# mbhall88/drprg

Measured on AMD Instinct MI355X. Metric: reads/sec (+ achieved HBM GB/s) predicting on mtb index, 1/2/4/8 GPUs, higher is better.
Workload: dtype u32

## Files before the change

### drprg_amd/_lib.py

```python
import ctypes as C
import os

_HERE = os.path.dirname(os.path.abspath(__file__))
LIB_PATH = os.environ.get("DRPRG_HIP_LIB") or os.path.join(_HERE, "lib", "libdrprg_hip.so")
PANDORA_EXE = os.path.join(_HERE, "bin", "pandora")


class MapOpts(C.Structure):
    _fields_ = [
        ("max_diff", C.c_int32),
        ("error_rate", C.c_double),
        ("min_cluster_size", C.c_uint32),
        ("illumina", C.c_int32),
        ("genome_size", C.c_uint64),
        ("genotyping_error_rate", C.c_double),
        ("kernel", C.c_int32),
        ("binomial", C.c_int32),
    ]


class AnnotateOpts(C.Structure):
    _fields_ = [
        ("min_covg", C.c_int32), ("max_covg", C.c_int32),
        ("min_strand_bias", C.c_float), ("min_gt_conf", C.c_float), ("min_frs", C.c_float),
# ... 70 lines not shown
    "drprg_hip_genotype": (C.c_int, [C.c_void_p, C.c_char_p, C.c_char_p, C.c_char_p]),
    "drprg_hip_genotype_info": (C.c_int, [C.c_void_p, C.POINTER(C.c_uint32)]),
    "drprg_hip_discover": (C.c_int, [C.c_void_p, C.c_char_p, C.c_char_p, C.c_char_p, C.POINTER(C.c_uint32)]),
    "drprg_hip_discover_reads": (C.c_int, [C.c_void_p, C.c_char_p, C.c_char_p, C.c_char_p, C.c_char_p, C.c_int, C.POINTER(C.c_uint32)]),
    "drprg_hip_update_prg": (C.c_int, [C.c_void_p, C.c_char_p, C.POINTER(C.c_uint32)]),
    "drprg_hip_update_prg_from_paths": (C.c_int, [C.c_void_p, C.c_char_p, C.c_char_p, C.POINTER(C.c_uint32)]),
    "drprg_hip_save_coverage": (C.c_int, [C.c_void_p, C.c_char_p, C.c_char_p]),
    "drprg_hip_load_coverage": (C.c_int, [C.c_void_p, C.c_char_p, C.c_char_p, C.POINTER(C.c_uint64)]),
    "drprg_hip_allele_stats": (C.c_int, [C.c_void_p, C.c_void_p, C.c_uint32, C.c_uint32, C.c_void_p, C.POINTER(C.c_double)]),
    "drprg_hip_genotype_site": (C.c_int, [C.c_void_p, C.c_void_p, C.c_void_p, C.c_uint32, C.c_double, C.c_double, C.c_void_p,
                                          C.POINTER(C.c_int32), C.POINTER(C.c_double)]),
    "drprg_hip_genotype_alleles": (C.c_int, [C.c_void_p, C.c_char_p]),
    "drprg_hip_estimate_parameters": (C.c_int, [C.c_void_p, C.c_uint64, C.c_uint64, C.c_uint64, C.c_uint32, C.c_int, C.c_double, C.c_int,
                                               C.POINTER(C.c_double)]),
    "drprg_hip_kmer_log_prob": (C.c_int, [C.c_int, C.c_double, C.c_double, C.c_double, C.c_uint32, C.c_uint32, C.c_uint32, C.POINTER(C.c_float)]),
    "drprg_hip_prob_threshold": (C.c_int, [C.c_void_p, C.c_uint64, C.POINTER(C.c_int)]),
    "drprg_hip_max_path": (C.c_int, [C.c_void_p, C.c_uint32, C.c_void_p, C.c_int, C.c_uint32, C.c_void_p, C.c_uint64, C.POINTER(C.c_uint64)]),
    "drprg_hip_path_base_coverage": (C.c_int, [C.c_void_p, C.c_uint32, C.c_void_p, C.c_uint64, C.c_void_p, C.c_void_p, C.c_uint64,
                                              C.POINTER(C.c_uint64)]),
    "drprg_hip_path_coverage_too_low": (C.c_int, [C.c_void_p, C.c_uint64, C.c_uint32]),
    "drprg_hip_coverage_model": (C.c_int, [C.c_void_p, C.POINTER(C.c_double)]),
    "drprg_hip_index_sizes": (C.c_int, [C.c_void_p, C.POINTER(C.c_uint64)]),
    "drprg_hip_filter_selfcheck": (C.c_int, [C.c_void_p, C.POINTER(C.c_uint64)]),
    "drprg_hip_device_tables": (C.c_int, [C.c_void_p, C.POINTER(C.c_uint64)]),
    "drprg_hip_index_export": (C.c_int, [C.c_void_p] + [C.c_void_p] * 7),
    "drprg_hip_prg_nodes": (C.c_int, [C.c_void_p, C.c_uint32, C.c_void_p, C.c_void_p, C.c_uint32, C.POINTER(C.c_uint32),
                                      C.POINTER(C.c_uint32)]),
    "drprg_hip_annotate": (C.c_int, [C.c_char_p, C.c_char_p, C.c_char_p, C.POINTER(AnnotateOpts), C.c_char_p, C.c_size_t]),
    "drprg_hip_vcf_to_bcf": (C.c_int, [C.c_char_p, C.c_char_p, C.c_char_p, C.c_size_t]),
    "drprg_hip_report_json": (C.c_int, [C.c_char_p, C.c_char_p, C.c_char_p, C.c_char_p, C.c_int, C.c_char_p, C.c_char_p,
                                        C.c_size_t]),
    "drprg_hip_kernel_timing": (C.c_int, [C.c_void_p, C.c_int, C.c_int, C.POINTER(C.c_double), C.POINTER(C.c_uint64)]),
    "drprg_hip_filter_schedule": (C.c_int, [C.c_void_p, C.POINTER(C.c_uint64)]),
    "drprg_hip_buffer_info": (C.c_int, [C.c_void_p, C.POINTER(C.c_uint64)]),
}


def load():
    if not os.path.exists(LIB_PATH):
        raise ImportError(
            f"{LIB_PATH} is missing: build the HIP extension first (`make` at the repo root or "
            "`python -c 'import __graft_entry__ as g; g.build()'`). There is no CPU fallback.")
    try:
        import torch
    except Exception:
        pass
# ... 10 lines not shown
```

### drprg_amd/csrc/capi.cpp

```cpp
#include <set>
#include <atomic>
#include <mutex>
#include <thread>
#include <fstream>
#include <cstdio>
#include "../../include/drprg_hip.h"
#include "fastx.h"
#include "genotype.h"
#include "bam.h"
#include "ingest.h"
#include "pgunzip.h"
#include "denovo.h"
#include "mapper.h"
#include "rccl_dyn.h"
#include "pack.h"
#include "read_qual_piece.h"
#include <algorithm>
#include <cstdlib>
#include <cstring>
#include <fcntl.h>
#include <functional>
#include <sys/mman.h>
#include <sys/stat.h>
#include <unistd.h>
// ... 1378 lines not shown
        al[a].gaps = gaps[a];
    }
    int g = 0;
    genotype_site(al, e, eps, g, *gt_conf);
    *gt = g;
    for (uint32_t a = 0; a < n_alleles; ++a) likelihood[a] = al[a].likelihood;
    return DRPRG_OK;
}

int drprg_hip_genotype_info(const drprg_hip_ctx* ctx, uint32_t out[4])
{
    if (!ctx || !out) return DRPRG_EINVAL;
    std::memcpy(out, ctx->ginfo, sizeof ctx->ginfo);
    return DRPRG_OK;
}

int drprg_hip_filter_selfcheck(const drprg_hip_ctx* ctx, uint64_t out[8])
{
    if (!ctx || !out) return DRPRG_EINVAL;
    ctx->index.filter_selfcheck(out);
    return DRPRG_OK;
}

int drprg_hip_index_sizes(const drprg_hip_ctx* ctx, uint64_t sizes[5])
{
    if (!ctx || !sizes) return DRPRG_EINVAL;
    const FlatIndex& f = ctx->index.flat;
    sizes[0] = f.keys.size();
    sizes[1] = f.rec_prg.size();
    sizes[2] = ctx->index.prgs.size();
    sizes[3] = f.total_knodes();
    sizes[4] = f.slot_key.size();
    return DRPRG_OK;
}

int drprg_hip_index_export(const drprg_hip_ctx* ctx, uint64_t* keys, uint32_t* rec_off, uint32_t* rec_prg, uint32_t* rec_knode,
    uint8_t* rec_strand, uint32_t* prg_min_path_len, uint32_t* prg_knode_base)
{
    if (!ctx) return DRPRG_EINVAL;
    const FlatIndex& f = ctx->index.flat;
    if (keys) std::memcpy(keys, f.keys.data(), f.keys.size() * sizeof(uint64_t));
    if (rec_off) std::memcpy(rec_off, f.rec_off.data(), f.rec_off.size() * sizeof(uint32_t));
    if (rec_prg) std::memcpy(rec_prg, f.rec_prg.data(), f.rec_prg.size() * sizeof(uint32_t));
    if (rec_knode) std::memcpy(rec_knode, f.rec_knode_global.data(), f.rec_knode_global.size() * sizeof(uint32_t));
    if (rec_strand) std::memcpy(rec_strand, f.rec_strand.data(), f.rec_strand.size());
    if (prg_min_path_len) std::memcpy(prg_min_path_len, f.min_path_len.data(), f.min_path_len.size() * sizeof(uint32_t));
// ... 246 lines not shown
```

### drprg_amd/csrc/common.h

```cpp
#pragma once
#include <cstdlib>
#include <cstdint>
#include <cstdio>
#include <stdexcept>
#include <string>
#include <vector>

namespace drprg {

struct Error : std::runtime_error {
    int code;
    Error(int c, const std::string& m) : std::runtime_error(m), code(c) {}
};

enum : int {
    DRPRG_OK = 0,
    DRPRG_EINVAL = -22,
    DRPRG_ENOENT = -2,
    DRPRG_EIO = -5,
    DRPRG_ENOMEM = -12,
    DRPRG_ENODEV = -19,
    DRPRG_EOVERFLOW = -75,
    DRPRG_EFORMAT = -84,
    DRPRG_ENODATA = -61,
// ... 10 lines not shown
    key = key ^ key >> 14;
    key = ((key + (key << 2)) + (key << 4)) & mask;
    key = key ^ key >> 28;
    key = (key + (key << 31)) & mask;
    return key;
}

inline int nt4(unsigned char c)
{
    switch (c) {
    case 'A': case 'a': return 0;
    case 'C': case 'c': return 1;
    case 'G': case 'g': return 2;
    case 'T': case 't': return 3;
    default: return 4;
    }
}

constexpr uint32_t BLOOM_C0 = 0xC2B2AFu;
constexpr uint32_t BLOOM_C1 = 0x9E3779u;
constexpr uint32_t BLOOM_C2 = 0x85EBCA6Bu;
constexpr uint32_t BLOOM_CR = 0xC2B2AE35u;
constexpr uint32_t BLOOMR_WBITS = 14;
constexpr uint32_t MID_BITMAP_WORDS = 1u << 19;
constexpr uint32_t MID_C_MAX_WBITS = 17;
inline uint32_t rc12_code(uint32_t x)
{
    uint32_t r = 0;
    for (int i = 0; i < 12; ++i) r |= (((x >> (2 * i)) & 3u) ^ 2u) << (2 * (11 - i));
    return r;
}
inline uint32_t canon12_code(uint32_t x)
{
    x &= 0xFFFFFFu;
    const uint32_t r = rc12_code(x);
    return x < r ? x : r;
}

inline bool canonical_kmer_hash(const char* s, int k, uint64_t& h, bool& strand)
{
    const uint64_t mask = kmer_mask(k);
    uint64_t f = 0, r = 0;
    for (int i = 0; i < k; ++i) {
        int c = nt4((unsigned char)s[i]);
        if (c > 3) return false;
        f = (f << 2) | (uint64_t)c;
// ... 24 lines not shown
```

### drprg_amd/csrc/index.cpp

```cpp
#include "index.h"
#include <algorithm>
#include <atomic>
#include <cerrno>
#include <cmath>
#include <cstdlib>
#include <fstream>
#include <sstream>
#include <sys/stat.h>
#include <thread>

namespace drprg {

static std::string dir_of(const std::string& p)
{
    size_t s = p.find_last_of('/');
    return s == std::string::npos ? std::string(".") : p.substr(0, s);
}

std::string PrgIndex::idx_path(const std::string& prg_file, int w, int k)
{
    return prg_file + ".k" + std::to_string(k) + ".w" + std::to_string(w) + ".idx";
}

std::string PrgIndex::gfa_path(const std::string& prg_file, const std::string& name, int w, int k)
// ... 13 lines not shown
    w = w_;
    k = k_;
    prgs = load_prg_file(prg_file);
    kgs.assign(prgs.size(), KmerGraph());
    std::atomic<size_t> next { 0 };
    std::string err;
    std::atomic<bool> failed { false };
    auto work = [&]() {
        for (size_t i; (i = next.fetch_add(1)) < prgs.size();) {
            try {
                kgs[i].build(prgs[i], w, k);
            } catch (const std::exception& e) {
                if (!failed.exchange(true)) err = e.what();
            }
        }
    };
    int nt = std::max(1, std::min<int>(threads, (int)prgs.size()));
    std::vector<std::thread> pool;
    for (int t = 1; t < nt; ++t) pool.emplace_back(work);
    work();
    for (auto& t : pool) t.join();
    if (failed) throw Error(DRPRG_EFORMAT, err);
    flatten(sw);
}

void PrgIndex::flatten(const Switches& sw)
{
    FlatIndex& f = flat;
    f = FlatIndex();
    f.knode_base.assign(prgs.size() + 1, 0);
    f.min_path_len.assign(prgs.size(), 0);
    struct Rec {
        uint64_t key;
        uint32_t prg, knode;
        uint8_t strand;
    };
    std::vector<Rec> recs;
    for (size_t p = 0; p < prgs.size(); ++p) {
        f.knode_base[p + 1] = f.knode_base[p] + (uint32_t)kgs[p].nodes.size();
        f.min_path_len[p] = kgs[p].shortest_path_length;
        const auto& nodes = kgs[p].nodes;
        for (size_t i = 1; i + 1 < nodes.size(); ++i)
            recs.push_back(Rec { nodes[i].hash, (uint32_t)p, nodes[i].id, (uint8_t)(nodes[i].strand ? 1 : 0) });
    }
    std::sort(recs.begin(), recs.end(), [](const Rec& a, const Rec& b) {
        if (a.key != b.key) return a.key < b.key;
// ... 50 lines not shown
        const uint32_t max_wbits = level0 ? MAX_WBITS - 1 : MAX_WBITS;
        uint32_t wbits = 8;
        while (wbits < max_wbits && (size_t(1) << wbits) * 5 < entries * 4) ++wbits;
        f.bloom_wbits = wbits;
        f.bloom.assign(size_t(1) << wbits, 0);
        const uint32_t wmask = (1u << wbits) - 1;
        const uint32_t kmask = (1u << (2 * k)) - 1;
        if (level0) {
            f.bloom0_wbits = L0_WBITS;
            f.bloom0.assign(size_t(1) << L0_WBITS, 0);
            f.bloom0f.assign(size_t(1) << L0_WBITS, 0);
            f.bloomr.assign(size_t(1) << BLOOMR_WBITS, 0);
        }
        const uint32_t wmask0 = (1u << L0_WBITS) - 1;
        for_each_code([&](uint32_t code) {
            const uint32_t x = code & kmask & 0xFFFFFFu;
            const uint32_t h = (uint32_t)((uint64_t)x * BLOOM_C1);
            f.bloom[(h >> 18) & wmask] |= (1u << (31 - (h & 31))) | (1u << (31 - ((h >> 8) & 31))) | (1u << (31 - ((x >> 16) & 31)));
            const uint32_t h2 = code * BLOOM_C2;
            f.bloom[h2 >> (32 - wbits)] |= (1u << (h2 & 31)) | (1u << ((h2 >> 5) & 31)) | (1u << ((h2 >> 10) & 31));
            if (level0) {
                const uint32_t hr = code * BLOOM_CR;
                f.bloomr[hr >> (32 - BLOOMR_WBITS)] |= (1u << (hr & 31)) | (1u << ((hr >> 5) & 31)) | (1u << ((hr >> 10) & 31)) | (1u << ((hr >> 15) & 31));
                const uint32_t hs = code * BLOOM_C2;
                f.bloom0f[hr >> (32 - L0_WBITS)] |= (1u << (hr & 31)) | (1u << ((hr >> 5) & 31)) | (1u << ((hr >> 10) & 31)) | (1u << (hs >> 27))
                    | (1u << ((hs >> 22) & 31)) | (1u << ((hs >> 17) & 31));
            }
            if (level0)
                for (int o = 0; o < 4; ++o) {
                    const uint32_t y = (code >> (2 * o)) & 0xFFFFFFu;
                    const uint32_t g = (uint32_t)((uint64_t)y * BLOOM_C0);
                    const uint32_t bits0 = (1u << (31 - (g & 31))) | (1u << (31 - ((g >> 8) & 31))) | (1u << (31 - ((y >> 16) & 31)));
                    f.bloom0[(g >> 17) & wmask0] |= bits0;
                    f.bloom0f[(g >> 17) & wmask0] |= bits0;
                }
        });
        if (level0) {
            uint32_t cw = 10;
            while (cw < MID_C_MAX_WBITS && (size_t(4) << cw) < 4 * entries) ++cw;
            f.blkc_wbits = cw;
            f.blkc.assign(size_t(4) << cw, 0);
            for_each_code([&](uint32_t code) {
                const uint32_t h = code * BLOOM_CR;
                for (int o = 0; o < 4; ++o) {
                    const uint32_t key = (code >> (2 * o)) & 0xFFFFFFu;
                    const uint32_t blk = (uint32_t)((uint64_t)key * BLOOM_C0) >> (32 - cw);
                    uint32_t* b = &f.blkc[(size_t)blk * 4];
                    b[0] |= 1u << (h >> 27);
                    b[1] |= 1u << ((h >> 22) & 31);
                    b[2] |= 1u << ((h >> 17) & 31);
                    b[3] |= 1u << ((h >> 12) & 31);
                }
            });
        }
    } else if (k == 15 && entries > 0 && recs.size() <= sw.mid_max_records) {
        f.mid_bitmap.assign(MID_BITMAP_WORDS, 0);
        for_each_code([&](uint32_t code) {
// ... 82 lines not shown
        out[4] = fill(f.mid0);
        out[5] = fill(f.mid_bitmap);
        out[6] = fill(f.midc);
        return;
    }
    if (!f.bloom_wbits) return;
    const uint32_t wmask = (1u << f.bloom_wbits) - 1, kmask = (1u << (2 * k)) - 1, wmask0 = f.bloom0_wbits ? (1u << f.bloom0_wbits) - 1 : 0;
    auto three = [](uint32_t word, uint32_t h, uint32_t x) {
        return ((word << (h & 31)) & (word << ((h >> 8) & 31)) & (word << ((x >> 16) & 31))) >> 31;
    };
    auto check = [&](uint32_t code) {
        ++out[0];
        if (f.bloom0_wbits) {
            bool any_miss = false;
            for (int o = 0; o < 4; ++o) {
                const uint32_t y = (code >> (2 * o)) & 0xFFFFFFu;
                const uint32_t g = (uint32_t)((uint64_t)y * BLOOM_C0);
                any_miss |= !three(f.bloom0[(g >> 17) & wmask0], g, y);
            }
            out[1] += any_miss;
            const uint32_t hr = code * BLOOM_CR, word = f.bloomr[hr >> (32 - BLOOMR_WBITS)];
            out[3] += !((word >> (hr & 31)) & (word >> ((hr >> 5) & 31)) & (word >> ((hr >> 10) & 31)) & (word >> ((hr >> 15) & 31)) & 1u);
            bool miss_f = false;
            for (int o = 0; o < 4; ++o) {
                const uint32_t y = (code >> (2 * o)) & 0xFFFFFFu;
                const uint32_t g = (uint32_t)((uint64_t)y * BLOOM_C0);
                miss_f |= !three(f.bloom0f[(g >> 17) & wmask0], g, y);
            }
            const uint32_t wf = f.bloom0f[hr >> (32 - f.bloom0_wbits)];
            const uint32_t hs = code * BLOOM_C2;
            miss_f |= !((wf >> (hr & 31)) & (wf >> ((hr >> 5) & 31)) & (wf >> ((hr >> 10) & 31)) & (wf >> (hs >> 27)) & (wf >> ((hs >> 22) & 31))
                & (wf >> ((hs >> 17) & 31)) & 1u);
            bool miss_blk = false;
            if (f.blkc_wbits)
                for (int o = 0; o < 4; ++o) {
                    const uint32_t key = (code >> (2 * o)) & 0xFFFFFFu;
                    const uint32_t* b = &f.blkc[(size_t)((uint32_t)((uint64_t)key * BLOOM_C0) >> (32 - f.blkc_wbits)) * 4];
                    miss_blk |= !((b[0] >> (hr >> 27)) & (b[1] >> ((hr >> 22) & 31)) & (b[2] >> ((hr >> 17) & 31)) & (b[3] >> ((hr >> 12) & 31)) & 1u);
                }
            out[7] += miss_f || miss_blk;
        }
        const uint32_t x = code & kmask & 0xFFFFFFu;
        const uint32_t h = (uint32_t)((uint64_t)x * BLOOM_C1);
        const uint32_t h2 = code * BLOOM_C2, w2 = f.bloom[h2 >> (32 - f.bloom_wbits)];
        const bool l1 = three(f.bloom[(h >> 18) & wmask], h, x);
        const bool l2 = (w2 >> (h2 & 31)) & (w2 >> ((h2 >> 5) & 31)) & (w2 >> ((h2 >> 10) & 31)) & 1u;
        out[2] += !(l1 && l2);
    };
    for (size_t p = 0; p < prgs.size(); ++p) {
        const auto& nodes = kgs[p].nodes;
        for (size_t i = 1; i + 1 < nodes.size(); ++i) {
            const std::string s = kpath_sequence(prgs[p], nodes[i].path);
            uint32_t fw = 0, rc = 0;
            for (int j = 0; j < k; ++j) {
                const uint32_t c = ((uint32_t)(unsigned char)s[(size_t)j] >> 1) & 3u;
                fw |= c << (2 * j);
                rc |= (c ^ 2u) << (2 * (k - 1 - j));
            }
            check(fw);
            check(rc);
        }
    }
    auto fill = [](const std::vector<uint32_t>& v) -> uint64_t {
        uint64_t bits = 0;
        for (uint32_t w : v) bits += (uint64_t)__builtin_popcount(w);
        return v.empty() ? 0 : bits * 1000 / (32 * (uint64_t)v.size());
    };
    out[4] = fill(f.bloom0);
    out[5] = fill(f.bloom);
    out[6] = fill(f.bloomr);
}

void PrgIndex::save(const std::string& prg_file) const
{
    std::string kdir = dir_of(prg_file) + "/kmer_prgs";
    if (mkdir(kdir.c_str(), 0777) != 0 && errno != EEXIST) throw Error(DRPRG_EIO, "cannot create " + kdir);
    for (size_t p = 0; p < prgs.size(); ++p) kgs[p].save_gfa(gfa_path(prg_file, prgs[p].name, w, k), prgs[p]);
    std::ofstream out(idx_path(prg_file, w, k));
    if (!out) throw Error(DRPRG_EIO, "cannot write " + idx_path(prg_file, w, k));
    const FlatIndex& f = flat;
    auto path_string = [&](uint32_t prg, uint32_t node) {
        std::ostringstream os;
        const KPath& kp = kgs[prg].nodes[node].path;
        os << kp.size() << "{";
        for (const PathPiece& pp : kp) {
            const uint32_t base = prgs[prg].nodes[pp.node].start;
            os << "[" << base + pp.off_start << ", " << base + pp.off_end << ")";
        }
        os << "}";
        return os.str();
    };
    out << f.keys.size() << "\n";
    for (size_t i = 0; i < f.keys.size(); ++i) {
// ... 66 lines not shown
```

### drprg_amd/csrc/index.h

```cpp
#pragma once
#include "kmergraph.h"
#include "switches.h"

namespace drprg {

struct MiniRecord {
    uint32_t prg;
    uint32_t knode;
    uint8_t strand;
};

struct FlatIndex {
    std::vector<uint64_t> keys;
    std::vector<uint32_t> rec_off;
    std::vector<uint32_t> rec_prg, rec_knode_global;
    std::vector<uint8_t> rec_strand;
    std::vector<uint32_t> knode_base;
    std::vector<uint32_t> min_path_len;
    uint32_t table_bits = 0;
    std::vector<uint64_t> slot_key;
    std::vector<uint32_t> slot_off, slot_cnt;
    uint32_t bloom_wbits = 0;
    std::vector<uint32_t> bloom;
    uint32_t bloom0_wbits = 0;
    std::vector<uint32_t> bloom0;
    std::vector<uint32_t> bloom0f;
    std::vector<uint32_t> bloomr;
    uint32_t midc_wbits = 0, mid0_bits = 0;
    std::vector<uint32_t> mid0, mid_bitmap, midc;
    uint32_t blkc_wbits = 0;
    std::vector<uint32_t> blkc;
    uint32_t total_knodes() const { return knode_base.empty() ? 0 : knode_base.back(); }
};

struct PrgIndex {
    int w = 0, k = 0;
    std::vector<LocalGraph> prgs;
    std::vector<KmerGraph> kgs;
    FlatIndex flat;
    void filter_selfcheck(uint64_t out[8]) const;

    static void check_wk(int w, int k);
    static void build_and_save(const std::string& prg_file, int w, int k, int threads, const Switches& sw);
    void build(const std::string& prg_file, int w, int k, int threads, const Switches& sw);
    void load(const std::string& prg_file, int w, int k, const Switches& sw);
    void save(const std::string& prg_file) const;

    static std::string idx_path(const std::string& prg_file, int w, int k);
    static std::string gfa_path(const std::string& prg_file, const std::string& name, int w, int k);

private:
    void flatten(const Switches& sw);
};

inline uint32_t table_slot(uint64_t key, uint32_t bits, bool narrow)
{
    if (narrow) return ((uint32_t)key * 0x9E3779B1u) >> (32 - bits);
    return (uint32_t)((key * 0x9E3779B97F4A7C15ULL) >> (64 - bits));
}

}
```

### drprg_amd/csrc/sketch_filter.hip

```cpp
#include "filter_common.h"
#include <algorithm>
#include <cstdint>
#include <type_traits>

namespace drprg {
namespace dev {

__device__ inline uint32_t pack16le(const uint4& in)
{
    constexpr uint32_t W = 0x40100401u;
    const uint32_t p0 = __builtin_amdgcn_udot4(in.x & 0x06060606u, W, 0u, false), p1 = __builtin_amdgcn_udot4(in.y & 0x06060606u, W, 0u, false);
    const uint32_t p2 = __builtin_amdgcn_udot4(in.z & 0x06060606u, W, 0u, false), p3 = __builtin_amdgcn_udot4(in.w & 0x06060606u, W, 0u, false);
    return ((p0 | (p1 << 8) | (p2 << 16)) >> 1) | (p3 << 23);
}


typedef __attribute__((address_space(3))) const uint32_t lds_cu32;
__device__ __forceinline__ uint32_t lds_at(uint32_t byte_addr) { return *(lds_cu32*)(uintptr_t)byte_addr; }
__device__ __forceinline__ uint32_t bloom_test(uint32_t word, uint32_t h, uint32_t x)
{
    uint32_t t2;
    asm("v_lshlrev_b32_sdwa %0, %1, %2 dst_sel:DWORD dst_unused:UNUSED_PAD src0_sel:BYTE_1 src1_sel:DWORD" : "=v"(t2) : "v"(h), "v"(word));
    return (word << (h & 31)) & t2 & (word << ((x >> 16) & 0xFF));
}

__device__ __forceinline__ uint32_t canon12_dev(uint32_t x)
{
    const uint32_t m = x & 0xFFFFFFu;
    const uint32_t r = __builtin_bitreverse32(x);
    const uint32_t rc = ((r >> 9) & 0x555555u) | (~(r >> 7) & 0xAAAAAAu);
    return m < rc ? m : rc;
}

template <bool SHORT_K, bool LEVEL0, bool FUSED = false, int MID = 0, bool PACKED = false>
__global__ __launch_bounds__(FT_THREADS) void sketch_filter_kernel(SketchArgs a, FilterWork fw)
{
    static_assert(FUSED == LEVEL0, "the level-0 form runs its second stage in this kernel");
    static_assert(MID == 0 || (LEVEL0 && FUSED), "the middle tier is a variant of the level-0 form with the second stage inside");
    extern __shared__ uint32_t s_dyn[];
    constexpr int G = filter_positions_per_lane(LEVEL0, PACKED), WPOS = 63 * G, NW = G / 16, NG = G / 4;
    constexpr uint32_t L12_BASE = LEVEL0 ? FT_L0_WORDS * 4u : 0u;
    constexpr bool CANON = MID == 1 || MID == 3;
    auto group_key = [](uint32_t x) -> uint32_t {
        if constexpr (CANON) return canon12_dev(x);
        else return x;
    };
    (void)group_key;
    constexpr uint32_t STAGE_RECORDS = 128, STAGE_CAP = STAGE_RECORDS - 1, STAGE_BASE_WORDS = FT_L0_WORDS;

    const int tid = threadIdx.x, lane = tid & 63;
    const int k = a.k;
    const int64_t n_bases = (int64_t)a.n_bases;
    const uint32_t n_words = 1u << fw.bloom_wbits;
    const uint32_t amask = (n_words - 1) << 2;
    const uint32_t amask0 = ((1u << fw.bloom0_wbits) - 1) << 2;
    const uint32_t kmask = (k < 16) ? ((1u << (2 * k)) - 1) : 0xFFFFFFFFu;
    const uint32_t kmask24 = kmask & 0xFFFFFFu;
    const int sh_w = 32 - (int)fw.bloom_wbits;
    const uint32_t sh_c = 32u - fw.midc_wbits;
    (void)sh_c;

    auto fill = [&](uint32_t lds_word0, const uint32_t* __restrict__ from, uint32_t n) {
        const uint4* __restrict__ src = reinterpret_cast<const uint4*>(from);
        uint4* dst = reinterpret_cast<uint4*>(s_dyn + lds_word0);
        for (uint32_t i = tid; i < n / 4; i += FT_THREADS) dst[i] = src[i];
    };
    if constexpr (LEVEL0) {
        constexpr int ROUNDS = FT_L0_WORDS / 4 / FT_THREADS;
        const uint4* __restrict__ src = reinterpret_cast<const uint4*>(fw.bloom0);
        uint4* dst = reinterpret_cast<uint4*>(s_dyn);
        uint4 v[ROUNDS];
#pragma unroll
        for (int r = 0; r < ROUNDS; ++r) v[r] = src[tid + r * FT_THREADS];
#pragma unroll
        for (int r = 0; r < ROUNDS; ++r) dst[tid + r * FT_THREADS] = v[r];
    }
    if (!LEVEL0) fill(L12_BASE / 4, fw.bloom, n_words);
    if (tid == 0 && (uint32_t)(uintptr_t)(__attribute__((address_space(3))) uint32_t*)s_dyn != 0u) atomicOr(a.overflow, 8u);
// ... 131 lines not shown
                        ra = stage[ia];                                                                                               \
                        ba = reinterpret_cast<const uint4*>(fw.midc)[(uint32_t)__umul24(group_key(__funnelshift_r(ra.z, ra.w, 6)), BLOOM_C0) >> sh_c];  \
                    }                                                                                                                 \
                    if (ib < lcnt) {                                                                                                  \
                        rb = stage[ib];                                                                                               \
                        bb = reinterpret_cast<const uint4*>(fw.midc)[(uint32_t)__umul24(group_key(__funnelshift_r(rb.z, rb.w, 6)), BLOOM_C0) >> sh_c]; \
                    }                                                                                                                 \
                    uint32_t ca = 0, cb = 0;                                                                                          \
                    DRPRG_BLOCK_TEST(ra, ba, ca);                            \
                    DRPRG_STAGE2_APPEND(ra, ca);                                                                                      \
                    if (c0 + 64 < lcnt) {                                                                           \
                        DRPRG_BLOCK_TEST(rb, bb, cb);                                                                                 \
                        DRPRG_STAGE2_APPEND(rb, cb);                                                                                  \
                    }                                                                                                                 \
                }                                                                                                                     \
            } else {                                                                                                                  \
                for (uint32_t c0 = 0; c0 < lcnt; c0 += 64) {                                                                          \
                    const uint32_t ri = c0 + (uint32_t)lane;                                                                          \
                    uint32_t cs = 0;                                                                                                  \
                    uint4 r = make_uint4(0, 0, 0, 0);                                                                                 \
                    if (ri < lcnt) {                                                                                                  \
                        r = stage[ri];                                                                                                \
                                                                     \
                        uint32_t hq[4], h2q[4], wq[4];                                                                                \
                        _Pragma("unroll") for (int q = 0; q < 4; ++q) {                                                               \
                            const uint32_t f = (q ? __funnelshift_r(r.z, r.w, 2 * q) : r.z) & kmask;                                  \
                            hq[q] = f * BLOOM_CR;                                                                                     \
                            h2q[q] = f * BLOOM_C2;                                                                                    \
                            wq[q] = lds_at((hq[q] >> 17) << 2);                                                                       \
                        }                                                                                                             \
                        __builtin_amdgcn_sched_barrier(0);      \
                        _Pragma("unroll") for (int q = 0; q < 4; ++q)                                                                 \
                            cs |= ((wq[q] >> (hq[q] & 31)) & (wq[q] >> ((hq[q] >> 5) & 31)) & (wq[q] >> ((hq[q] >> 10) & 31)) & (wq[q] >> (h2q[q] >> 27)) \
                                      & (wq[q] >> ((h2q[q] >> 22) & 31)) & (wq[q] >> ((h2q[q] >> 17) & 31)) & 1u) << q;               \
                    }                                                                                                                 \
                    DRPRG_STAGE2_APPEND(r, cs);                                                                                       \
                }                                                                                                                     \
            }                                                                                                                         \
            __builtin_amdgcn_wave_barrier();                                                                                          \
            lcnt = 0;                                                                                                                 \
        }                                                                                                                             \
    } while (0)
    auto close_slice = [&]() {
        if constexpr (FUSED) DRPRG_SECOND_STAGE();
        if (lane == 0) {
            const uint32_t kept = wcur < cap_cur ? wcur : cap_cur;
            fw.slice_count[slice] = kept;
            fw.slice_base[slice] = base_cur;
            fw.slice_cap[slice] = cap_cur;
            if (wcur > cap_cur) atomicOr(a.overflow, 4u);
            if (kept) atomicAdd(&fw.super_count[slice / FT_SUPER], kept);
        }
    };

    auto process = [&](uint32_t t, const Pair& p) {
        uint32_t wv[NW + 1];
        if constexpr (PACKED) {
            wv[0] = p.x;
            wv[1] = p.y;
            if constexpr (NW == 4) {
                wv[2] = p.z;
                wv[3] = p.w;
            }
        } else {
            wv[0] = pack16le(p.a);
            wv[1] = pack16le(p.b);
        }
        wv[NW] = __builtin_amdgcn_update_dpp(0u, wv[0], 0x130 , 0xF, 0xF, true);
        const uint32_t wa = wv[0], wb = wv[1], wc = wv[2];
        (void)wa; (void)wb; (void)wc;
        if constexpr (LEVEL0) {
            uint32_t grp = 0, xs[NG], hs[NG], ws[NG];
#pragma unroll
            for (int g = 0; g < NG; ++g) {
                const int j = 4 * g + 3;
                const uint32_t lo = wv[j >> 4], hi = wv[(j >> 4) + 1];
                xs[g] = __builtin_amdgcn_alignbit(hi, lo, 2 * (j & 15));
                if constexpr (CANON) xs[g] = canon12_dev(xs[g]);
                hs[g] = __umul24(xs[g], BLOOM_C0);
                ws[g] = lds_at((hs[g] >> 15) & amask0);
            }
#pragma unroll
            for (int g = NG - 1; g >= 0; --g)
                grp = __builtin_amdgcn_alignbit(grp, MID == 1 ? ws[g] << (hs[g] & 31) : bloom_test(ws[g], hs[g], xs[g]), 31);
            grp &= lane_keep;
            if constexpr (CANON) {
                uint32_t bw[NG];
#pragma unroll
                for (int g = 0; g < NG; ++g) {
                    bw[g] = 0;
                    if (grp & (1u << g)) bw[g] = fw.mid_bitmap[xs[g] >> 5];
                }
                uint32_t keep = 0;
#pragma unroll
                for (int g = 0; g < NG; ++g) keep |= ((bw[g] >> (xs[g] & 31)) & 1u) << g;
                grp &= keep;
            }
            const uint32_t cnt = (uint32_t)__popc(grp);
            const uint64_t b0 = __ballot(cnt & 1u), b1 = __ballot(cnt & 2u), b2 = __ballot(cnt & 4u), b3 = __ballot(cnt & 8u);
            const uint64_t b4 = NG > 8 ? __ballot(cnt & 16u) : 0ull;
            if (b0 | b1 | b2 | b3 | b4) {
                auto below = [&](uint64_t m) { return __builtin_amdgcn_mbcnt_hi((uint32_t)(m >> 32), __builtin_amdgcn_mbcnt_lo((uint32_t)m, 0u)); };
                auto lanes_below = [&]() { return below(b0) + 2u * below(b1) + 4u * below(b2) + 8u * below(b3) + (NG > 8 ? 16u * below(b4) : 0u); };
                const uint32_t total = (uint32_t)(__popcll(b0) + 2 * __popcll(b1) + 4 * __popcll(b2) + 8 * __popcll(b3) + (NG > 8 ? 16 * __popcll(b4) : 0));
                const uint64_t base = (uint64_t)t * WPOS + (uint64_t)lane * G;
                auto record = [&](int g) {
                    const int q = g >> 2;
// ... 355 lines not shown
```

### drprg_amd/pandora.py

```python
import ctypes as C
import os
import re

import numpy as np

from ._lib import MapOpts, lib

MTB_GENOME_SIZE = 4411532


class DependencyError(RuntimeError):

    def __init__(self, kind, message, code=0):
        super().__init__(f"{kind}: {message}")
        self.kind = kind
        self.code = code


def _check(rc, ctx=None):
    if rc != 0:
        msg = lib.drprg_hip_last_error(ctx)
        raise DependencyError("ProcessError", (msg or b"").decode() or f"error {rc}", code=-rc)


# ... 246 lines not shown
    def load_coverage(self, path, tag):
        rc = lib.drprg_hip_load_coverage(self._h, os.fsencode(path), tag.encode(), None)
        if rc == -2:
            return False
        _check(rc, self._h)
        return True

    def genotype_alleles(self, out_tsv):
        _check(lib.drprg_hip_genotype_alleles(self._h, os.fsencode(out_tsv)), self._h)
        out = {}
        for line in open(out_tsv):
            if line.startswith("#"):
                continue
            chrom, pos, a, n, nodes = line.rstrip("\n").split("\t")
            out[(chrom, int(pos), int(a))] = np.array([int(x) for x in nodes.split(",") if x], dtype=np.int64)
        return out

    def filter_selfcheck(self):
        out = (C.c_uint64 * 8)()
        _check(lib.drprg_hip_filter_selfcheck(self._h, out), self._h)
        names = ("codes", "level0_false_negatives", "level12_false_negatives", "stage2_false_negatives", "level0_fill_permille",
                 "level12_fill_permille", "stage2_fill_permille", "shared_array_false_negatives")
        return dict(zip(names, (int(x) for x in out)))

    def table_tier(self):
        out = (C.c_uint64 * 6)()
        _check(lib.drprg_hip_device_tables(self._h, out), self._h)
        return dict(pbloom_words=int(out[0]), table_bytes=int(out[1]), lds_filter_bytes=int(out[2]), kernel=int(out[3]),
                    l2_filter_bytes=int(out[4]), sketch_form=int(out[5]))

    def export_index(self):
        keys = np.zeros(self.n_keys, dtype=np.uint64)
        rec_off = np.zeros(self.n_keys + 1, dtype=np.uint32)
        rec_prg = np.zeros(self.n_records, dtype=np.uint32)
        rec_knode = np.zeros(self.n_records, dtype=np.uint32)
        rec_strand = np.zeros(self.n_records, dtype=np.uint8)
        min_path_len = np.zeros(self.n_prgs, dtype=np.uint32)
        knode_base = np.zeros(self.n_prgs + 1, dtype=np.uint32)
        _check(lib.drprg_hip_index_export(self._h, _ptr(keys), _ptr(rec_off), _ptr(rec_prg), _ptr(rec_knode), _ptr(rec_strand),
                                          _ptr(min_path_len), _ptr(knode_base)), self._h)
        return dict(keys=keys, rec_off=rec_off, rec_prg=rec_prg, rec_knode=rec_knode, rec_strand=rec_strand,
                    min_path_len=min_path_len, knode_base=knode_base)

    def prg_nodes(self, prg):
        n, ns = C.c_uint32(), C.c_uint32()
        _check(lib.drprg_hip_prg_nodes(self._h, prg, None, None, 0, C.byref(n), C.byref(ns)), self._h)
# ... 174 lines not shown
```

### include/drprg_hip.h

```cpp
#ifndef DRPRG_HIP_H
#define DRPRG_HIP_H

#include <stddef.h>
#include <stdint.h>

#ifdef __cplusplus
extern "C" {
#endif

typedef struct drprg_hip_ctx drprg_hip_ctx;

#define DRPRG_HIP_MAP_OPTS_SIZE 48
typedef struct drprg_hip_map_opts {
    int32_t max_diff;
    double error_rate;
    uint32_t min_cluster_size;
    int32_t illumina;
    uint64_t genome_size;
    double genotyping_error_rate;
    int32_t kernel;
    int32_t binomial;
} drprg_hip_map_opts;

int drprg_hip_index(const char* prg_file, int w, int k, int threads);
// ... 67 lines not shown
int drprg_hip_resident_info(drprg_hip_ctx* ctx, uint64_t out[4]);
int drprg_hip_subsample(drprg_hip_ctx* ctx, uint64_t target_bases, uint64_t seed, uint64_t out[4]);
int drprg_hip_set_ordered_ingest(drprg_hip_ctx* ctx, int on);
int drprg_hip_subsample_flags(drprg_hip_ctx* ctx, uint8_t* flags, uint64_t n);
int drprg_hip_set_read_filter(drprg_hip_ctx* ctx, uint64_t min_len, uint64_t max_len, uint32_t min_qual_milli);
int drprg_hip_read_filter_info(drprg_hip_ctx* ctx, uint64_t out[8]);
int drprg_hip_read_filter_device(drprg_hip_ctx* ctx, const void* d_qual, uint32_t qual_bias, const void* d_offsets, uint64_t n_reads, uint64_t n_bases,
    void* d_sums, void* d_flags, uint64_t out[4], void* hip_stream);
int drprg_hip_select_reads(drprg_hip_ctx* ctx, const uint64_t* anchors, uint64_t n_anchors, uint32_t A, uint64_t window_bytes, uint8_t* bases,
    uint64_t bases_cap, uint64_t* offsets, uint64_t* ids, uint64_t reads_cap, uint64_t out[2]);

int drprg_hip_update_prg(drprg_hip_ctx* ctx, const char* out_prg, uint32_t* n_applied);
int drprg_hip_update_prg_from_paths(drprg_hip_ctx* ctx, const char* denovo_paths, const char* out_prg, uint32_t* n_applied);

int drprg_hip_save_coverage(drprg_hip_ctx* ctx, const char* path, const char* tag);
int drprg_hip_load_coverage(drprg_hip_ctx* ctx, const char* path, const char* tag, uint64_t counters[8]);

int drprg_hip_allele_stats(const uint32_t* fwd, const uint32_t* rev, uint32_t n, uint32_t min_kmer_covg, uint32_t out[6], double* gaps);
int drprg_hip_genotype_site(const uint32_t* mean_fwd, const uint32_t* mean_rev, const double* gaps, uint32_t n_alleles, double e,
    double eps, double* likelihood, int32_t* gt, double* gt_conf);
int drprg_hip_genotype_alleles(drprg_hip_ctx* ctx, const char* out_tsv);

int drprg_hip_filter_selfcheck(const drprg_hip_ctx* ctx, uint64_t out[8]);
int drprg_hip_estimate_parameters(const uint32_t* kmer_covg, uint64_t n, uint64_t clusters, uint64_t loci, uint32_t global_covg, int k,
    double e_rate, int bin, double out[10]);
int drprg_hip_kmer_log_prob(int use_bin, double nb_p, double nb_r, double bin_p, uint32_t fwd, uint32_t rev, uint32_t locus_reads, float* out);
int drprg_hip_prob_threshold(const float* logp, uint64_t n, int* out);
int drprg_hip_max_path(const drprg_hip_ctx* ctx, uint32_t prg, const float* logp, int thresh, uint32_t max_kmers_to_average, uint32_t* path,
    uint64_t cap, uint64_t* n_path);
int drprg_hip_path_base_coverage(const drprg_hip_ctx* ctx, uint32_t prg, const uint32_t* path, uint64_t n_path, const uint32_t* covg2,
    uint32_t* out, uint64_t cap, uint64_t* n_out);
int drprg_hip_path_coverage_too_low(const uint32_t* base_covg, uint64_t n, uint32_t global_covg);
int drprg_hip_coverage_model(const drprg_hip_ctx* ctx, double out[12]);

int drprg_hip_index_sizes(const drprg_hip_ctx* ctx, uint64_t sizes[5]);
int drprg_hip_index_export(const drprg_hip_ctx* ctx, uint64_t* keys, uint32_t* rec_off, uint32_t* rec_prg,
    uint32_t* rec_knode, uint8_t* rec_strand, uint32_t* prg_min_path_len, uint32_t* prg_knode_base);

int drprg_hip_device_tables(drprg_hip_ctx* ctx, uint64_t out[6]);

int drprg_hip_prg_nodes(const drprg_hip_ctx* ctx, uint32_t prg, uint32_t* starts, uint32_t* ends, uint32_t cap,
    uint32_t* n_nodes, uint32_t* n_sites);

typedef struct drprg_hip_annotate_opts {
    int32_t min_covg, max_covg;
    float min_strand_bias, min_gt_conf, min_frs;
// ... 23 lines not shown
```

Baseline: 21.69 billion.

## Widen shared level-0/stage-2 bloom array to 64-bit blocks

```diff
diff --git a/drprg_amd/_lib.py b/drprg_amd/_lib.py
--- a/drprg_amd/_lib.py
+++ b/drprg_amd/_lib.py
@@ -116,6 +116,8 @@
     "drprg_hip_coverage_model": (C.c_int, [C.c_void_p, C.POINTER(C.c_double)]),
     "drprg_hip_index_sizes": (C.c_int, [C.c_void_p, C.POINTER(C.c_uint64)]),
     "drprg_hip_filter_selfcheck": (C.c_int, [C.c_void_p, C.POINTER(C.c_uint64)]),
+    "drprg_hip_filter_sample": (C.c_int, [C.c_void_p, C.c_uint64, C.c_uint64, C.POINTER(C.c_uint64)]),
+    "drprg_hip_filter_arrays": (C.c_int, [C.c_void_p, C.c_void_p, C.c_void_p, C.c_uint64, C.POINTER(C.c_uint64)]),
     "drprg_hip_device_tables": (C.c_int, [C.c_void_p, C.POINTER(C.c_uint64)]),
     "drprg_hip_index_export": (C.c_int, [C.c_void_p] + [C.c_void_p] * 7),
     "drprg_hip_prg_nodes": (C.c_int, [C.c_void_p, C.c_uint32, C.c_void_p, C.c_void_p, C.c_uint32, C.POINTER(C.c_uint32),
diff --git a/drprg_amd/csrc/capi.cpp b/drprg_amd/csrc/capi.cpp
--- a/drprg_amd/csrc/capi.cpp
+++ b/drprg_amd/csrc/capi.cpp
@@ -1424,6 +1424,25 @@
     return DRPRG_OK;
 }
 
+int drprg_hip_filter_sample(const drprg_hip_ctx* ctx, uint64_t seed, uint64_t n, uint64_t out[8])
+{
+    if (!ctx || !out) return DRPRG_EINVAL;
+    ctx->index.filter_sample(seed, n, out);
+    return DRPRG_OK;
+}
+
+int drprg_hip_filter_arrays(const drprg_hip_ctx* ctx, uint32_t* shared, uint32_t* level0, uint64_t capacity_words, uint64_t* n_words)
+{
+    if (!ctx || !n_words) return DRPRG_EINVAL;
+    const FlatIndex& f = ctx->index.flat;
+    *n_words = f.bloom0f.size();
+    if (!shared && !level0) return DRPRG_OK;
+    if (capacity_words < f.bloom0f.size() || f.bloom0.size() != f.bloom0f.size()) return DRPRG_EINVAL;
+    if (shared) std::copy(f.bloom0f.begin(), f.bloom0f.end(), shared);
+    if (level0) std::copy(f.bloom0.begin(), f.bloom0.end(), level0);
+    return DRPRG_OK;
+}
+
 int drprg_hip_index_sizes(const drprg_hip_ctx* ctx, uint64_t sizes[5])
 {
     if (!ctx || !sizes) return DRPRG_EINVAL;
diff --git a/drprg_amd/csrc/common.h b/drprg_amd/csrc/common.h
--- a/drprg_amd/csrc/common.h
+++ b/drprg_amd/csrc/common.h
@@ -56,6 +56,9 @@
 constexpr uint32_t BLOOM_C2 = 0x85EBCA6Bu;
 constexpr uint32_t BLOOM_CR = 0xC2B2AE35u;
 constexpr uint32_t BLOOMR_WBITS = 14;
+constexpr int L0F_BLOCK_BITS = 64;
+constexpr int L0F_KEY_BITS = 4;
+static_assert((L0F_BLOCK_BITS == 32 && L0F_KEY_BITS == 3) || (L0F_BLOCK_BITS == 64 && L0F_KEY_BITS == 4), "shared-array geometry");
 constexpr uint32_t MID_BITMAP_WORDS = 1u << 19;
 constexpr uint32_t MID_C_MAX_WBITS = 17;
 inline uint32_t rc12_code(uint32_t x)
diff --git a/drprg_amd/csrc/index.cpp b/drprg_amd/csrc/index.cpp
--- a/drprg_amd/csrc/index.cpp
+++ b/drprg_amd/csrc/index.cpp
@@ -59,6 +59,29 @@
     for (auto& t : pool) t.join();
     if (failed) throw Error(DRPRG_EFORMAT, err);
     flatten(sw);
+}
+
+struct SharedBits {
+    uint32_t word, lo, hi;
+};
+static SharedBits shared_level0_bits(uint32_t y, uint32_t wbits)
+{
+    const uint32_t g = (uint32_t)((uint64_t)y * BLOOM_C0), w = (g >> 17) & ((1u << wbits) - 1);
+    auto bit = [](uint32_t sel) { return 1u << (31 - (sel & 31)); };
+    if (L0F_BLOCK_BITS == 32) return { w, bit(g) | bit(g >> 8) | bit(y >> 16), 0u };
+    return { w & ~1u, bit(g) | bit(g >> 8), bit(y >> 16) | bit(y >> 8) };
+}
+static SharedBits shared_stage2_bits(uint32_t code, uint32_t wbits)
+{
+    const uint32_t hr = code * BLOOM_CR, hs = code * BLOOM_C2, w = hr >> (32 - wbits);
+    const uint32_t lo = (1u << (hr & 31)) | (1u << ((hr >> 5) & 31)) | (1u << ((hr >> 10) & 31));
+    const uint32_t hi = (1u << (hs >> 27)) | (1u << ((hs >> 22) & 31)) | (1u << ((hs >> 17) & 31));
+    if (L0F_BLOCK_BITS == 32) return { w, lo | hi, 0u };
+    return { w & ~1u, lo, hi };
+}
+static bool shared_holds(const std::vector<uint32_t>& arr, const SharedBits& b)
+{
+    return (arr[b.word] & b.lo) == b.lo && (L0F_BLOCK_BITS == 32 || (arr[b.word + 1] & b.hi) == b.hi);
 }
 
 void PrgIndex::flatten(const Switches& sw)
@@ -155,9 +178,9 @@
             if (level0) {
                 const uint32_t hr = code * BLOOM_CR;
                 f.bloomr[hr >> (32 - BLOOMR_WBITS)] |= (1u << (hr & 31)) | (1u << ((hr >> 5) & 31)) | (1u << ((hr >> 10) & 31)) | (1u << ((hr >> 15) & 31));
-                const uint32_t hs = code * BLOOM_C2;
-                f.bloom0f[hr >> (32 - L0_WBITS)] |= (1u << (hr & 31)) | (1u << ((hr >> 5) & 31)) | (1u << ((hr >> 10) & 31)) | (1u << (hs >> 27))
-                    | (1u << ((hs >> 22) & 31)) | (1u << ((hs >> 17) & 31));
+                const SharedBits sb = shared_stage2_bits(code, L0_WBITS);
+                f.bloom0f[sb.word] |= sb.lo;
+                f.bloom0f[sb.word + (L0F_BLOCK_BITS == 64)] |= sb.hi;
             }
             if (level0)
                 for (int o = 0; o < 4; ++o) {
@@ -165,7 +188,9 @@
                     const uint32_t g = (uint32_t)((uint64_t)y * BLOOM_C0);
                     const uint32_t bits0 = (1u << (31 - (g & 31))) | (1u << (31 - ((g >> 8) & 31))) | (1u << (31 - ((y >> 16) & 31)));
                     f.bloom0[(g >> 17) & wmask0] |= bits0;
-                    f.bloom0f[(g >> 17) & wmask0] |= bits0;
+                    const SharedBits sb = shared_level0_bits(y, L0_WBITS);
+                    f.bloom0f[sb.word] |= sb.lo;
+                    f.bloom0f[sb.word + (L0F_BLOCK_BITS == 64)] |= sb.hi;
                 }
         });
         if (level0) {
@@ -294,15 +319,8 @@
             const uint32_t hr = code * BLOOM_CR, word = f.bloomr[hr >> (32 - BLOOMR_WBITS)];
             out[3] += !((word >> (hr & 31)) & (word >> ((hr >> 5) & 31)) & (word >> ((hr >> 10) & 31)) & (word >> ((hr >> 15) & 31)) & 1u);
             bool miss_f = false;
-            for (int o = 0; o < 4; ++o) {
-                const uint32_t y = (code >> (2 * o)) & 0xFFFFFFu;
-                const uint32_t g = (uint32_t)((uint64_t)y * BLOOM_C0);
-                miss_f |= !three(f.bloom0f[(g >> 17) & wmask0], g, y);
-            }
-            const uint32_t wf = f.bloom0f[hr >> (32 - f.bloom0_wbits)];
-            const uint32_t hs = code * BLOOM_C2;
-            miss_f |= !((wf >> (hr & 31)) & (wf >> ((hr >> 5) & 31)) & (wf >> ((hr >> 10) & 31)) & (wf >> (hs >> 27)) & (wf >> ((hs >> 22) & 31))
-                & (wf >> ((hs >> 17) & 31)) & 1u);
+            for (int o = 0; o < 4; ++o) miss_f |= !shared_holds(f.bloom0f, shared_level0_bits((code >> (2 * o)) & 0xFFFFFFu, f.bloom0_wbits));
+            miss_f |= !shared_holds(f.bloom0f, shared_stage2_bits(code, f.bloom0_wbits));
             bool miss_blk = false;
             if (f.blkc_wbits)
                 for (int o = 0; o < 4; ++o) {
@@ -341,6 +359,41 @@
     out[4] = fill(f.bloom0);
     out[5] = fill(f.bloom);
     out[6] = fill(f.bloomr);
+}
+
+void PrgIndex::filter_sample(uint64_t seed, uint64_t n, uint64_t out[8]) const
+{
+    for (int i = 0; i < 8; ++i) out[i] = 0;
+    const FlatIndex& f = flat;
+    if (!f.bloom0_wbits || f.bloom0f.empty()) return;
+    auto next = [&seed]() {
+        uint64_t z = (seed += 0x9E3779B97F4A7C15ull);
+        z = (z ^ (z >> 30)) * 0xBF58476D1CE4E5B9ull;
+        z = (z ^ (z >> 27)) * 0x94D049BB133111EBull;
+        return z ^ (z >> 31);
+    };
+    auto fill = [](const std::vector<uint32_t>& v) -> uint64_t {
+        uint64_t bits = 0;
+        for (uint32_t w : v) bits += (uint64_t)__builtin_popcount(w);
+        return bits * 1000000 / (32 * (uint64_t)v.size());
+    };
+    const uint32_t wmask0 = (1u << f.bloom0_wbits) - 1, kmask = (1u << (2 * k)) - 1;
+    out[0] = n;
+    out[1] = fill(f.bloom0f);
+    out[4] = fill(f.bloom0);
+    for (uint64_t i = 0; i < n; ++i) {
+        const uint64_t r = next();
+        const uint32_t y = (uint32_t)r & 0xFFFFFFu, code = (uint32_t)(r >> 32) & kmask;
+        out[2] += shared_holds(f.bloom0f, shared_level0_bits(y, f.bloom0_wbits));
+        out[3] += shared_holds(f.bloom0f, shared_stage2_bits(code, f.bloom0_wbits));
+        const uint32_t g = (uint32_t)((uint64_t)y * BLOOM_C0), word = f.bloom0[(g >> 17) & wmask0];
+        out[5] += ((word << (g & 31)) & (word << ((g >> 8) & 31)) & (word << ((y >> 16) & 31))) >> 31;
+        if (f.blkc_wbits) {
+            const uint32_t h = code * BLOOM_CR;
+            const uint32_t* b = &f.blkc[(size_t)((uint32_t)((uint64_t)(code & 0xFFFFFFu) * BLOOM_C0) >> (32 - f.blkc_wbits)) * 4];
+            out[6] += (b[0] >> (h >> 27)) & (b[1] >> ((h >> 22) & 31)) & (b[2] >> ((h >> 17) & 31)) & (b[3] >> ((h >> 12) & 31)) & 1u;
+        }
+    }
 }
 
 void PrgIndex::save(const std::string& prg_file) const
diff --git a/drprg_amd/csrc/index.h b/drprg_amd/csrc/index.h
--- a/drprg_amd/csrc/index.h
+++ b/drprg_amd/csrc/index.h
@@ -39,6 +39,7 @@
     std::vector<KmerGraph> kgs;
     FlatIndex flat;
     void filter_selfcheck(uint64_t out[8]) const;
+    void filter_sample(uint64_t seed, uint64_t n, uint64_t out[8]) const;
 
     static void check_wk(int w, int k);
     static void build_and_save(const std::string& prg_file, int w, int k, int threads, const Switches& sw);
diff --git a/drprg_amd/csrc/sketch_filter.hip b/drprg_amd/csrc/sketch_filter.hip
--- a/drprg_amd/csrc/sketch_filter.hip
+++ b/drprg_amd/csrc/sketch_filter.hip
@@ -22,6 +22,17 @@
     uint32_t t2;
     asm("v_lshlrev_b32_sdwa %0, %1, %2 dst_sel:DWORD dst_unused:UNUSED_PAD src0_sel:BYTE_1 src1_sel:DWORD" : "=v"(t2) : "v"(h), "v"(word));
     return (word << (h & 31)) & t2 & (word << ((x >> 16) & 0xFF));
+}
+
+typedef uint32_t u32x2 __attribute__((ext_vector_type(2)));
+typedef __attribute__((address_space(3))) const u32x2 lds_cu64;
+__device__ __forceinline__ u32x2 lds64_at(uint32_t byte_addr) { return *(lds_cu64*)(uintptr_t)byte_addr; }
+__device__ __forceinline__ uint32_t bloom_test64(u32x2 blk, uint32_t h, uint32_t x)
+{
+    uint32_t t1, t3;
+    asm("v_lshlrev_b32_sdwa %0, %1, %2 dst_sel:DWORD dst_unused:UNUSED_PAD src0_sel:BYTE_1 src1_sel:DWORD" : "=v"(t1) : "v"(h), "v"(blk.x));
+    asm("v_lshlrev_b32_sdwa %0, %1, %2 dst_sel:DWORD dst_unused:UNUSED_PAD src0_sel:BYTE_1 src1_sel:DWORD" : "=v"(t3) : "v"(x), "v"(blk.y));
+    return (blk.x << (h & 31)) & t1 & (blk.y << ((x >> 16) & 0xFF)) & t3;
 }
 
 __device__ __forceinline__ uint32_t canon12_dev(uint32_t x)
@@ -41,6 +52,7 @@
     constexpr int G = filter_positions_per_lane(LEVEL0, PACKED), WPOS = 63 * G, NW = G / 16, NG = G / 4;
     constexpr uint32_t L12_BASE = LEVEL0 ? FT_L0_WORDS * 4u : 0u;
     constexpr bool CANON = MID == 1 || MID == 3;
+    constexpr bool WIDE = MID == 0 && LEVEL0 && L0F_BLOCK_BITS == 64;
     auto group_key = [](uint32_t x) -> uint32_t {
         if constexpr (CANON) return canon12_dev(x);
         else return x;
@@ -53,7 +65,7 @@
     const int64_t n_bases = (int64_t)a.n_bases;
     const uint32_t n_words = 1u << fw.bloom_wbits;
     const uint32_t amask = (n_words - 1) << 2;
-    const uint32_t amask0 = ((1u << fw.bloom0_wbits) - 1) << 2;
+    const uint32_t amask0 = (((1u << fw.bloom0_wbits) - 1) << 2) & (WIDE ? ~7u : ~0u);
     const uint32_t kmask = (k < 16) ? ((1u << (2 * k)) - 1) : 0xFFFFFFFFu;
     const uint32_t kmask24 = kmask & 0xFFFFFFu;
     const int sh_w = 32 - (int)fw.bloom_wbits;
@@ -231,17 +243,24 @@
                     if (ri < lcnt) {                                                                                                  \
                         r = stage[ri];                                                                                                \
                                                                      \
-                        uint32_t hq[4], h2q[4], wq[4];                                                                                \
+                                         \
+                        uint32_t hq[4], h2q[4], wq[4], vq[4];                                                                         \
                         _Pragma("unroll") for (int q = 0; q < 4; ++q) {                                                               \
                             const uint32_t f = (q ? __funnelshift_r(r.z, r.w, 2 * q) : r.z) & kmask;                                  \
                             hq[q] = f * BLOOM_CR;                                                                                     \
                             h2q[q] = f * BLOOM_C2;                                                                                    \
-                            wq[q] = lds_at((hq[q] >> 17) << 2);                                                                       \
+                            if constexpr (WIDE) {                                                                                     \
+                                const u32x2 b2 = lds64_at((hq[q] >> 18) << 3);                                                        \
+                                wq[q] = b2.x;                                                                                         \
+                                vq[q] = b2.y;                                                                                         \
+                            } else {                                                                                                  \
+                                wq[q] = vq[q] = lds_at((hq[q] >> 17) << 2);                                                           \
+                            }                                                                                                         \
                         }                                                                                                             \
                         __builtin_amdgcn_sched_barrier(0);      \
                         _Pragma("unroll") for (int q = 0; q < 4; ++q)                                                                 \
-                            cs |= ((wq[q] >> (hq[q] & 31)) & (wq[q] >> ((hq[q] >> 5) & 31)) & (wq[q] >> ((hq[q] >> 10) & 31)) & (wq[q] >> (h2q[q] >> 27)) \
-                                      & (wq[q] >> ((h2q[q] >> 22) & 31)) & (wq[q] >> ((h2q[q] >> 17) & 31)) & 1u) << q;               \
+                            cs |= ((wq[q] >> (hq[q] & 31)) & (wq[q] >> ((hq[q] >> 5) & 31)) & (wq[q] >> ((hq[q] >> 10) & 31)) & (vq[q] >> (h2q[q] >> 27)) \
+                                      & (vq[q] >> ((h2q[q] >> 22) & 31)) & (vq[q] >> ((h2q[q] >> 17) & 31)) & 1u) << q;               \
                     }                                                                                                                 \
                     DRPRG_STAGE2_APPEND(r, cs);                                                                                       \
                 }                                                                                                                     \
@@ -279,7 +298,9 @@
         const uint32_t wa = wv[0], wb = wv[1], wc = wv[2];
         (void)wa; (void)wb; (void)wc;
         if constexpr (LEVEL0) {
-            uint32_t grp = 0, xs[NG], hs[NG], ws[NG];
+            using Block = typename std::conditional<WIDE, u32x2, uint32_t>::type;
+            uint32_t grp = 0, xs[NG], hs[NG];
+            Block ws[NG];
 #pragma unroll
             for (int g = 0; g < NG; ++g) {
                 const int j = 4 * g + 3;
@@ -287,11 +308,16 @@
                 xs[g] = __builtin_amdgcn_alignbit(hi, lo, 2 * (j & 15));
                 if constexpr (CANON) xs[g] = canon12_dev(xs[g]);
                 hs[g] = __umul24(xs[g], BLOOM_C0);
-                ws[g] = lds_at((hs[g] >> 15) & amask0);
-            }
-#pragma unroll
-            for (int g = NG - 1; g >= 0; --g)
-                grp = __builtin_amdgcn_alignbit(grp, MID == 1 ? ws[g] << (hs[g] & 31) : bloom_test(ws[g], hs[g], xs[g]), 31);
+                if constexpr (WIDE) ws[g] = lds64_at((hs[g] >> 15) & amask0);
+                else ws[g] = lds_at((hs[g] >> 15) & amask0);
+            }
+#pragma unroll
+            for (int g = NG - 1; g >= 0; --g) {
+                uint32_t t;
+                if constexpr (WIDE) t = bloom_test64(ws[g], hs[g], xs[g]);
+                else t = MID == 1 ? ws[g] << (hs[g] & 31) : bloom_test(ws[g], hs[g], xs[g]);
+                grp = __builtin_amdgcn_alignbit(grp, t, 31);
+            }
             grp &= lane_keep;
             if constexpr (CANON) {
                 uint32_t bw[NG];
diff --git a/drprg_amd/pandora.py b/drprg_amd/pandora.py
--- a/drprg_amd/pandora.py
+++ b/drprg_amd/pandora.py
@@ -292,6 +292,24 @@
         names = ("codes", "level0_false_negatives", "level12_false_negatives", "stage2_false_negatives", "level0_fill_permille",
                  "level12_fill_permille", "stage2_fill_permille", "shared_array_false_negatives")
         return dict(zip(names, (int(x) for x in out)))
+
+    def filter_sample(self, seed, n):
+        out = (C.c_uint64 * 8)()
+        _check(lib.drprg_hip_filter_sample(self._h, seed, n, out), self._h)
+        v = [int(x) for x in out]
+        if not v[0]:
+            return {}
+        return dict(n=v[0], shared_fill=v[1] / 1e6, shared_level0_pass=v[2] / v[0], shared_stage2_pass=v[3] / v[0],
+                    level0_fill=v[4] / 1e6, level0_pass=v[5] / v[0], block_stage2_pass=v[6] / v[0])
+
+    def filter_arrays(self):
+        n = C.c_uint64()
+        _check(lib.drprg_hip_filter_arrays(self._h, None, None, 0, C.byref(n)), self._h)
+        if not n.value:
+            return None, None
+        shared, level0 = np.zeros(n.value, dtype=np.uint32), np.zeros(n.value, dtype=np.uint32)
+        _check(lib.drprg_hip_filter_arrays(self._h, _ptr(shared), _ptr(level0), n.value, C.byref(n)), self._h)
+        return shared, level0
 
     def table_tier(self):
         out = (C.c_uint64 * 6)()
diff --git a/include/drprg_hip.h b/include/drprg_hip.h
--- a/include/drprg_hip.h
+++ b/include/drprg_hip.h
@@ -113,6 +113,8 @@
 int drprg_hip_genotype_alleles(drprg_hip_ctx* ctx, const char* out_tsv);
 
 int drprg_hip_filter_selfcheck(const drprg_hip_ctx* ctx, uint64_t out[8]);
+int drprg_hip_filter_sample(const drprg_hip_ctx* ctx, uint64_t seed, uint64_t n, uint64_t out[8]);
+int drprg_hip_filter_arrays(const drprg_hip_ctx* ctx, uint32_t* shared, uint32_t* level0, uint64_t capacity_words, uint64_t* n_words);
 int drprg_hip_estimate_parameters(const uint32_t* kmer_covg, uint64_t n, uint64_t clusters, uint64_t loci, uint32_t global_covg, int k,
     double e_rate, int bin, double out[10]);
 int drprg_hip_kmer_log_prob(int use_bin, double nb_p, double nb_r, double bin_p, uint32_t fwd, uint32_t rev, uint32_t locus_reads, float* out);
```

After: 22.09 billion, median of 6. No clear change (+1.8%).
